# ShuangXieIrene/ssds.pytorch

Hardware: AMD Instinct MI355X
Metric: images/sec (fwd+decode+NMS) SSD-MobileNetV2@512 (higher is better)
Workload: dtype bf16

## Files before the change

### ssds.pytorch_amd/csrc/ssdk_mbk.hip

```cpp
#include "ssdk_common.h"
#include "ssdk_flow_common.h"
#include "ssdk_scan.h"

namespace ssdk {

struct MbkParams {
  const u16* x;
  u16* y;
  const unsigned char* img;
  int N, H, W, Ho, Wo, Cin, Chid, Cout, residual;
  int pairs, halves;
  unsigned items;
  unsigned long long* dbg;
  unsigned wave_mask, pair_mask;
};

template <int KS, int NW, int NCHW, int NFO>
struct MbkGeo {
  static constexpr int NP = (NCHW + 1) / 2;
  static constexpr int PAIR_KB = 2 * KS + NFO;
  static constexpr int MISC_KB = (NCHW * 384 + 1023) / 1024;
  static constexpr int m_be = 0, m_wd = NCHW * 64, m_bd = NCHW * (64 + 288);
  static constexpr int SPB_KB = 2;
  static_assert(NFO * 128 <= SPB_KB * 1024, "projection BN block");
  __host__ __device__ static size_t weights(int halves) { return (size_t)halves * NW * NP * PAIR_KB * 1024; }
  __host__ __device__ static size_t misc_off(int halves) { return weights(halves); }
  __host__ __device__ static size_t spb_off(int halves) { return misc_off(halves) + (size_t)NW * MISC_KB * 1024; }
  __host__ __device__ static size_t bytes(int halves) { return spb_off(halves) + (size_t)halves * SPB_KB * 1024; }
};

template <int S, int NS>
struct MbkItem {
  static constexpr int NXS = NS * S;
  static constexpr int NR = S + 3;
};

template <int S, int NS, int KS, int NW, int NCHW, int NFO>
struct MbkLds {
  using G = MbkGeo<KS, NW, NCHW, NFO>;
  using I = MbkItem<S, NS>;
  static constexpr int FT = 2 * NS * NFO;
  static constexpr int XF = FT % 5 == 0 ? 5 : (FT % 8 == 0 ? 8 : 4);
  static_assert(FT % XF == 0, "exchange rounds");
  static constexpr int xt = 0;
  static constexpr int misc = xt + I::NR * I::NXS * KS * 1024;
  static constexpr int spb = misc + NW * G::MISC_KB * 1024;
  static constexpr int xch = spb + G::SPB_KB * 1024;
  static constexpr int bytes = xch + NW * XF * 1024;
};

__device__ __forceinline__ void mbk_mfma_guard() {
  __builtin_amdgcn_sched_barrier(0);
  asm volatile("s_nop 15\n\ts_nop 3" ::: "memory");
  __builtin_amdgcn_sched_barrier(0);
}
__device__ __forceinline__ void mbk_valu_guard() {
  __builtin_amdgcn_sched_barrier(0);
  asm volatile("s_nop 3" ::: "memory");
  __builtin_amdgcn_sched_barrier(0);
}
__device__ __forceinline__ u32 fl_from_left2(u32 cur, u32 prev) {
  const int old = __builtin_amdgcn_update_dpp(0, (int)prev, 0x121, 0xf, 0xf, true);
  return (u32)__builtin_amdgcn_update_dpp(old, (int)cur, 0x111, 0xf, 0xf, false);
}
__device__ __forceinline__ u32 fl_from_right2(u32 cur, u32 next) {
  const int old = __builtin_amdgcn_update_dpp(0, (int)next, 0x12f, 0xf, 0xf, true);
  return (u32)__builtin_amdgcn_update_dpp(old, (int)cur, 0x101, 0xf, 0xf, false);
}

template <int DT, int S, int NS, int KS, int NW, int NCHW, int NFO, bool DBG = false>
__global__ __launch_bounds__(64 * NW, 2) void mbk_kernel(const MbkParams p) {
  using L = MbkLds<S, NS, KS, NW, NCHW, NFO>;
  using G = MbkGeo<KS, NW, NCHW, NFO>;
  using I = MbkItem<S, NS>;
  constexpr int NR = I::NR, NXS = I::NXS, NE = NR * NXS;
  constexpr int XF = L::XF, FT = L::FT, NP = G::NP, PAIR_KB = G::PAIR_KB;
  constexpr int NO = 2 * NS;
  constexpr bool ODD = (NCHW & 1) != 0;
  constexpr int ROUNDS = FT / XF;
  extern __shared__ __attribute__((aligned(16))) unsigned char smem[];
  const u32 tid = threadIdx.x, lane = tid & 63u;
  const u32 fr = lane & 15u, fg = lane >> 4;
  const int wv = __builtin_amdgcn_readfirstlane((int)(tid >> 6));
  const int Cin = p.Cin, Cout = p.Cout, H = p.H, W = p.W, Ho = p.Ho, Wo = p.Wo;

  const u32 item = blockIdx.x;
  const int half = (int)(item % (u32)p.halves);
  const u32 rem = item / (u32)p.halves;
  const int n = (int)(rem / (u32)p.pairs), rp = (int)(rem % (u32)p.pairs);
  const int oy0 = 2 * rp;
  const int iy0 = S * oy0 - 1;
  const int co_base = half * 16 * NFO;
  const u16* ximg = p.x + (size_t)n * H * W * Cin;
  const bool stamp = p.dbg != nullptr && blockIdx.x == 0 && tid == 0;
  if (stamp) p.dbg[0] = __builtin_readcyclecounter();

  const u32x4* wimg = reinterpret_cast<const u32x4*>(p.img + ((size_t)(half * NW + wv) * NP) * ((size_t)PAIR_KB * 1024)) + lane;
  u32x4 wa[KS], wb[KS];
#pragma unroll
  for (int ks = 0; ks < KS; ++ks) {
    wa[ks] = wimg[(size_t)ks * 64];
    wb[ks] = wimg[(size_t)(KS + ks) * 64];
  }

  for (int e = wv; e < NE; e += NW) {
    const int r = e / NXS, xs = e % NXS;
    int iy = iy0 + r;
    iy = iy < 0 ? 0 : (iy > H - 1 ? H - 1 : iy);
    const int col = S == 1 ? 16 * xs + (int)fr : 2 * (16 * (xs >> 1) + (int)fr) + (xs & 1);
    const u16* src = ximg + ((size_t)iy * W + col) * Cin + fg * 8;
#pragma unroll
    for (int ks = 0; ks < KS; ++ks)
      __builtin_amdgcn_global_load_lds((glb_u8*)(src + ks * 32), (lds_u8*)(smem + L::xt + (e * KS + ks) * 1024), 16, 0, 0);
  }
  {
    const unsigned char* src = p.img + G::misc_off(p.halves) + (size_t)wv * (G::MISC_KB * 1024) + lane * 16;
#pragma unroll
    for (int k = 0; k < G::MISC_KB; ++k)
      __builtin_amdgcn_global_load_lds((glb_u8*)(src + k * 1024), (lds_u8*)(smem + L::misc + (wv * G::MISC_KB + k) * 1024), 16, 0, 0);
  }
  if (wv == 0) {
    const unsigned char* src = p.img + G::spb_off(p.halves) + (size_t)half * (G::SPB_KB * 1024) + lane * 16;
#pragma unroll
    for (int k = 0; k < G::SPB_KB; ++k)
      __builtin_amdgcn_global_load_lds((glb_u8*)(src + k * 1024), (lds_u8*)(smem + L::spb + k * 1024), 16, 0, 0);
  }
  asm volatile("s_waitcnt vmcnt(0)" ::: "memory");
  __syncthreads();
  if (stamp) p.dbg[1] = __builtin_readcyclecounter();

  fl_f2 hi[NR];
#pragma unroll
  for (int r = 0; r < NR; ++r) {
    const float k = ((unsigned)(iy0 + r) < (unsigned)H) ? kFlSixth : 0.f;
    hi[r] = fl_f2{k, k};
  }

  f32x4 yacc[NO][NFO];
#pragma unroll
  for (int o = 0; o < NO; ++o)
#pragma unroll
    for (int f = 0; f < NFO; ++f) yacc[o][f] = f32x4{0.f, 0.f, 0.f, 0.f};

  const unsigned char* xt = smem + L::xt + lane * 16;
  const unsigned char* mc = smem + L::misc + wv * (G::MISC_KB * 1024);

  auto chunk = [&](int c, const u32x4 (&w)[KS], u32 (&dout)[NO][2]) {
    const f32x4 bv = *reinterpret_cast<const f32x4*>(mc + G::m_be + (c * 4 + (int)fg) * 16);
    f32x4 e[NE];
#pragma unroll
    for (int i = 0; i < NE; ++i) e[i] = bv;
#pragma unroll
    for (int ks = 0; ks < KS; ++ks) {
      u32x4 xf[NE];
#pragma unroll
      for (int i = 0; i < NE; ++i) xf[i] = *reinterpret_cast<const u32x4*>(xt + (i * KS + ks) * 1024);
#pragma unroll
      for (int i = 0; i < NE; ++i) e[i] = fl_mfma<DT>(w[ks], xf[i], e[i]);
    }
    uint2 wt[9];
#pragma unroll
    for (int t = 0; t < 9; ++t) wt[t] = *reinterpret_cast<const uint2*>(mc + G::m_wd + ((c * 9 + t) * 4 + (int)fg) * 8);
    const uint2 bdi = *reinterpret_cast<const uint2*>(mc + G::m_bd + (c * 4 + (int)fg) * 8);
    mbk_mfma_guard();
    u32 ew[NR][NXS][2];
#pragma unroll
    for (int r = 0; r < NR; ++r)
#pragma unroll
      for (int xs = 0; xs < NXS; ++xs) {
        ew[r][xs][0] = fl_unit_pack(e[r * NXS + xs][0], e[r * NXS + xs][1], hi[r]);
        ew[r][xs][1] = fl_unit_pack(e[r * NXS + xs][2], e[r * NXS + xs][3], hi[r]);
      }
#pragma unroll
    for (int o = 0; o < 2; ++o)
#pragma unroll
      for (int j = 0; j < NS; ++j) {
        fl_h2 s[2] = {fl_as_h2(bdi.x), fl_as_h2(bdi.y)};
#pragma unroll
        for (int ky = 0; ky < 3; ++ky) {
          const int r = S * o + ky;
          const uint2 w0 = wt[ky * 3], w1 = wt[ky * 3 + 1], w2 = wt[ky * 3 + 2];
#pragma unroll
          for (int wd = 0; wd < 2; ++wd) {
            u32 tl, tc, tr;
            if constexpr (S == 1) {
              tc = ew[r][j][wd];
              tl = j == 0 ? fl_from_left(tc) : fl_from_left2(tc, ew[r][j > 0 ? j - 1 : 0][wd]);
              tr = j == NS - 1 ? fl_from_right(tc) : fl_from_right2(tc, ew[r][j < NS - 1 ? j + 1 : j][wd]);
            } else {
              const u32 odd = ew[r][2 * j + 1][wd];
              tc = ew[r][2 * j][wd];
              tl = j == 0 ? fl_from_left(odd) : fl_from_left2(odd, ew[r][j > 0 ? 2 * j - 1 : 1][wd]);
              tr = odd;
            }
            const u32 ww0 = wd ? w0.y : w0.x, ww1 = wd ? w1.y : w1.x, ww2 = wd ? w2.y : w2.x;
            s[wd] = __builtin_elementwise_fma(fl_as_h2(tl), fl_as_h2(ww0), s[wd]);
            s[wd] = __builtin_elementwise_fma(fl_as_h2(tc), fl_as_h2(ww1), s[wd]);
            if (ky == 2) s[wd] = fl_fma_clamp01(fl_as_h2(tr), fl_as_h2(ww2), s[wd]);
            else s[wd] = __builtin_elementwise_fma(fl_as_h2(tr), fl_as_h2(ww2), s[wd]);
          }
        }
        dout[o * NS + j][0] = fl_as_u32(s[0]);
        dout[o * NS + j][1] = fl_as_u32(s[1]);
      }
  };

  constexpr int FH = NFO / 2;
  for (int t = 0; t < NP; ++t) {
    const u32x4* wp = wimg + (size_t)t * (PAIR_KB * 64);
    const bool last = t == NP - 1;
    const u32x4* wn = wimg + (size_t)(last ? t : t + 1) * (PAIR_KB * 64);
    u32 d0[NO][2], d1[NO][2];
    u32x4 wf0[FH], wf1[NFO - FH];
#pragma unroll
    for (int f = 0; f < FH; ++f) wf0[f] = wp[(size_t)(2 * KS + f) * 64];
    chunk(2 * t, wa, d0);
    __builtin_amdgcn_sched_barrier(0);
    u32x4 na[KS];
#pragma unroll
    for (int ks = 0; ks < KS; ++ks) na[ks] = wn[(size_t)ks * 64];
#pragma unroll
    for (int f = FH; f < NFO; ++f) wf1[f - FH] = wp[(size_t)(2 * KS + f) * 64];
    if (!(ODD && last)) {
      chunk(2 * t + 1, wb, d1);
    } else {
#pragma unroll
      for (int o = 0; o < NO; ++o) d1[o][0] = d1[o][1] = 0u;
    }
    __builtin_amdgcn_sched_barrier(0);
    u32x4 nb[KS];
#pragma unroll
    for (int ks = 0; ks < KS; ++ks) nb[ks] = wn[(size_t)(KS + ks) * 64];
    u32x4 db[NO];
#pragma unroll
    for (int o = 0; o < NO; ++o) db[o] = u32x4{d0[o][0], d0[o][1], d1[o][0], d1[o][1]};
    if constexpr (DBG) {
      if (!((p.pair_mask >> t) & 1u) || !((p.wave_mask >> wv) & 1u)) {
#pragma unroll
        for (int o = 0; o < NO; ++o) db[o] = u32x4{0u, 0u, 0u, 0u};
      }
    }
    mbk_valu_guard();
#pragma unroll
    for (int f = 0; f < NFO; ++f)
#pragma unroll
      for (int o = 0; o < NO; ++o)
        yacc[o][f] = fl_mfma<SSDK_F16>(f < FH ? wf0[f < FH ? f : 0] : wf1[f >= FH ? f - FH : 0], db[o], yacc[o][f]);
    __builtin_amdgcn_sched_barrier(0);
#pragma unroll
    for (int ks = 0; ks < KS; ++ks) {
      wa[ks] = na[ks];
      wb[ks] = nb[ks];
    }
  }
  if (stamp) p.dbg[2] = __builtin_readcyclecounter();

  unsigned char* xb = smem + L::xch;
  const unsigned char* spb = smem + L::spb;
  constexpr int GPW = (XF + NW - 1) / NW;
  uint2 resv[ROUNDS][GPW];
#pragma unroll
  for (int R = 0; R < ROUNDS; ++R)
#pragma unroll
    for (int gg = 0; gg < GPW; ++gg) {
      const int g = wv + gg * NW, q = R * XF + g, oj = q / NFO, f = q % NFO;
      const int oy = oy0 + oj / NS, ox = 16 * (oj % NS) + (int)fr, co = co_base + f * 16 + (int)fg * 4;
      resv[R][gg] = make_uint2(0u, 0u);
      if (S == 1 && p.residual && g < XF && oy < Ho && co < Cout)
        resv[R][gg] = *reinterpret_cast<const uint2*>(ximg + ((size_t)oy * W + ox) * Cin + co);
    }
#pragma unroll
  for (int R = 0; R < ROUNDS; ++R) {
#pragma unroll
    for (int g = 0; g < XF; ++g) {
      const int q = R * XF + g, oj = q / NFO, f = q % NFO;
      *reinterpret_cast<f32x4*>(xb + ((wv * XF + g) * 64 + (int)lane) * 16) = yacc[oj][f];
    }
    __syncthreads();
#pragma unroll
    for (int gg = 0; gg < GPW; ++gg) {
      const int g = wv + gg * NW;
      if (g < XF) {
        const int q = R * XF + g, oj = q / NFO, f = q % NFO;
        f32x4 y = *reinterpret_cast<const f32x4*>(xb + ((0 * XF + g) * 64 + (int)lane) * 16);
#pragma unroll
        for (int w2 = 1; w2 < NW; ++w2) {
          const f32x4 t2 = *reinterpret_cast<const f32x4*>(xb + ((w2 * XF + g) * 64 + (int)lane) * 16);
          y = y + t2;
        }
        const int oy = oy0 + oj / NS, ox = 16 * (oj % NS) + (int)fr;
        const int co = co_base + f * 16 + (int)fg * 4;
        if (oy < Ho && co < Cout) {
          const f32x4 spv = *reinterpret_cast<const f32x4*>(spb + (f * 4 + (int)fg) * 32);
          const f32x4 bpv = *reinterpret_cast<const f32x4*>(spb + (f * 4 + (int)fg) * 32 + 16);
          u32 h01 = fl_pack2<DT>(fmaf(y[0], spv[0], bpv[0]), fmaf(y[1], spv[1], bpv[1]));
          u32 h23 = fl_pack2<DT>(fmaf(y[2], spv[2], bpv[2]), fmaf(y[3], spv[3], bpv[3]));
          if (S == 1 && p.residual) {
            const uint2 xr = resv[R][gg];
            h01 = fl_pack2<DT>(fl_from16<DT>(h01 & 0xffffu) + fl_from16<DT>(xr.x & 0xffffu), fl_from16<DT>(h01 >> 16) + fl_from16<DT>(xr.x >> 16));
            h23 = fl_pack2<DT>(fl_from16<DT>(h23 & 0xffffu) + fl_from16<DT>(xr.y & 0xffffu), fl_from16<DT>(h23 >> 16) + fl_from16<DT>(xr.y >> 16));
          }
          u16* yrow = p.y + (((size_t)n * Ho + oy) * Wo + ox) * Cout;
          *reinterpret_cast<uint2*>(yrow + co) = make_uint2(h01, h23);
        }
      }
    }
    if (R + 1 < ROUNDS) __syncthreads();
  }
  if (stamp) p.dbg[3] = __builtin_readcyclecounter();
}

template <int DT, int S, int NS, int KS, int NW, int NCHW, int NFO, bool DBG = false>
static void mbk_launch(const MbkParams& p, hipStream_t stream) {
  constexpr int lds = MbkLds<S, NS, KS, NW, NCHW, NFO>::bytes;
  static_assert(lds <= 160 * 1024, "LDS");
  (void)hipFuncSetAttribute(reinterpret_cast<const void*>(&mbk_kernel<DT, S, NS, KS, NW, NCHW, NFO, DBG>),
                            hipFuncAttributeMaxDynamicSharedMemorySize, lds);
  hipLaunchKernelGGL((mbk_kernel<DT, S, NS, KS, NW, NCHW, NFO, DBG>), dim3(p.items), dim3(64 * NW), lds, stream, p);
}

constexpr int kMbkNW = 4;
struct MbkInst {
  int s, ns, ks, nchw, nfo;
};
static const MbkInst kMbkInst[] = {{1, 1, 5, 15, 10}, {2, 1, 3, 9, 10}, {1, 2, 2, 6, 4}, {1, 2, 2, 6, 6}, {1, 2, 3, 9, 6},
                                   {2, 2, 1, 3, 4}, {1, 4, 1, 3, 2}};

static int mbk_find(int stride, int Wo, int Cin, int Chid, int Cout, int nw, int* halves) {
  if (nw != kMbkNW || Cin % 32 || Chid % 16 || Cout % 16 || Wo % 16) return -1;
  const int ks = Cin / 32, nch = Chid / 16, nchw = (nch + nw - 1) / nw, ns = Wo / 16;
  for (int i = 0; i < (int)(sizeof(kMbkInst) / sizeof(kMbkInst[0])); ++i) {
    const MbkInst& k = kMbkInst[i];
    if (k.s == stride && k.ns == ns && k.ks == ks && k.nchw == nchw && Cout % (16 * k.nfo) == 0) {
      if (halves) *halves = Cout / (16 * k.nfo);
      return i;
    }
  }
  return -1;
}

static size_t mbk_bytes(int inst, int halves) {
  switch (inst) {
    case 0: return MbkGeo<5, kMbkNW, 15, 10>::bytes(halves);
    case 1: return MbkGeo<3, kMbkNW, 9, 10>::bytes(halves);
    case 2: return MbkGeo<2, kMbkNW, 6, 4>::bytes(halves);
    case 3: return MbkGeo<2, kMbkNW, 6, 6>::bytes(halves);
    case 4: return MbkGeo<3, kMbkNW, 9, 6>::bytes(halves);
    case 5: return MbkGeo<1, kMbkNW, 3, 4>::bytes(halves);
    case 6: return MbkGeo<1, kMbkNW, 3, 2>::bytes(halves);
  }
  return 0;
}

template <int DT>
static void mbk_dispatch(const MbkParams& p, int inst, hipStream_t stream) {
  const bool dbg = p.wave_mask != ~0u || p.pair_mask != ~0u;
  switch (inst) {
    case 0: dbg ? mbk_launch<DT, 1, 1, 5, kMbkNW, 15, 10, true>(p, stream) : mbk_launch<DT, 1, 1, 5, kMbkNW, 15, 10>(p, stream); break;
    case 1: mbk_launch<DT, 2, 1, 3, kMbkNW, 9, 10>(p, stream); break;
    case 2: mbk_launch<DT, 1, 2, 2, kMbkNW, 6, 4>(p, stream); break;
    case 3: mbk_launch<DT, 1, 2, 2, kMbkNW, 6, 6>(p, stream); break;
    case 4: mbk_launch<DT, 1, 2, 3, kMbkNW, 9, 6>(p, stream); break;
    case 5: mbk_launch<DT, 2, 2, 1, kMbkNW, 3, 4>(p, stream); break;
    case 6: mbk_launch<DT, 1, 4, 1, kMbkNW, 3, 2>(p, stream); break;
  }
}

int launch_mbk(const ssdk_mbconv_desc* d, hipStream_t stream) {
  static const int env = getenv("SSDK_MBK") ? atoi(getenv("SSDK_MBK")) : 1;
  const int variant = d->variant;
  if ((!env && variant != 3) || (variant != 0 && variant != 3)) return 1;
  if (d->stem || !d->w_image || d->image_nw < 1 || (d->stride != 1 && d->stride != 2)) return 1;
  const int Ho = (d->H + 2 - 3) / d->stride + 1, Wo = (d->W + 2 - 3) / d->stride + 1;
  if (d->W != Wo * d->stride) return 1;
  int halves = 0;
  const int inst = mbk_find(d->stride, Wo, d->Cin, d->Chid, d->Cout, d->image_nw, &halves);
  if (inst < 0 || (size_t)d->w_image_bytes < mbk_bytes(inst, halves) || ((uintptr_t)d->w_image & 15)) return 1;
  if (env != 1 && variant != 3 && !((env >> (inst + 1)) & 1)) return 1;
  const int pairs = (Ho + 1) / 2;
  const long items = (long)halves * d->N * pairs;
  constexpr int env_min = 256;
  if (items < env_min && variant != 3) return 1;
  MbkParams p;
  p.x = (const u16*)d->x;
  p.y = (u16*)d->y;
  p.img = (const unsigned char*)d->w_image;
  p.N = d->N;
  p.H = d->H;
  p.W = d->W;
  p.Ho = Ho;
  p.Wo = Wo;
  p.Cin = d->Cin;
  p.Chid = d->Chid;
  p.Cout = d->Cout;
  p.residual = d->residual;
  p.pairs = pairs;
  p.halves = halves;
  p.items = (unsigned)items;
  p.dbg = nullptr;
  p.wave_mask = p.pair_mask = ~0u;
  if (const char* m = getenv("SSDK_MBK_MASKS")) {
    unsigned a = ~0u, b = ~0u;
    if (sscanf(m, "%x,%x", &a, &b) == 2) {
      p.wave_mask = a;
      p.pair_mask = b;
    }
  }
  static const int env_dbg = getenv("SSDK_MB_DBG") ? atoi(getenv("SSDK_MB_DBG")) : 0;
  static unsigned long long* dbg_dev = nullptr;
  if (env_dbg) {
    if (!dbg_dev) (void)hipMalloc(&dbg_dev, 8 * sizeof(unsigned long long));
    p.dbg = dbg_dev;
  }
  if (d->dtype == SSDK_BF16) mbk_dispatch<SSDK_BF16>(p, inst, stream);
  else mbk_dispatch<SSDK_F16>(p, inst, stream);
  if (env_dbg) {
    unsigned long long h[4];
    (void)hipStreamSynchronize(stream);
    (void)hipMemcpy(h, dbg_dev, sizeof(h), hipMemcpyDeviceToHost);
    fprintf(stderr, "[mbk dbg] Cin=%d Chid=%d Cout=%d s=%d W=%d items=%ld : setup %llu loop %llu exchange %llu\n", d->Cin, d->Chid,
            d->Cout, d->stride, d->W, items, h[1] - h[0], h[2] - h[1], h[3] - h[2]);
  }
  return 0;
}

}

extern "C" size_t ssdk_mbk_image_bytes(int Cin, int Chid, int Cout, int stride, int Wo, int nw, int* nfo) {
  int halves = 0;
  const int inst = ssdk::mbk_find(stride, Wo, Cin, Chid, Cout, nw, &halves);
  if (inst < 0) return 0;
  if (nfo) *nfo = ssdk::kMbkInst[inst].nfo;
  return ssdk::mbk_bytes(inst, halves);
}
```

Baseline: 65130.

## Make MobileNet block kernel persistent with double-buffered input tile prefetch

```diff
diff --git a/ssds.pytorch_amd/csrc/ssdk_mbk.hip b/ssds.pytorch_amd/csrc/ssdk_mbk.hip
--- a/ssds.pytorch_amd/csrc/ssdk_mbk.hip
+++ b/ssds.pytorch_amd/csrc/ssdk_mbk.hip
@@ -11,6 +11,7 @@
   int N, H, W, Ho, Wo, Cin, Chid, Cout, residual;
   int pairs, halves;
   unsigned items;
+  unsigned grid;
   unsigned long long* dbg;
   unsigned wave_mask, pair_mask;
 };
@@ -39,15 +40,57 @@
 struct MbkLds {
   using G = MbkGeo<KS, NW, NCHW, NFO>;
   using I = MbkItem<S, NS>;
+  static constexpr int kHalfCu = 80 * 1024;
   static constexpr int FT = 2 * NS * NFO;
-  static constexpr int XF = FT % 5 == 0 ? 5 : (FT % 8 == 0 ? 8 : 4);
+  static constexpr int XF1 = FT % 5 == 0 ? 5 : (FT % 8 == 0 ? 8 : 4);
+  static constexpr int xt_bytes = I::NR * I::NXS * KS * 1024;
+  static constexpr int fixed = (NW * G::MISC_KB + G::SPB_KB) * 1024;
+  static constexpr bool two_xf1 = 2 * xt_bytes + fixed + NW * XF1 * 1024 <= kHalfCu;
+  static constexpr bool two_xf4 = FT % 4 == 0 && 2 * xt_bytes + fixed + NW * 4 * 1024 <= kHalfCu;
+  static constexpr int NXB = (two_xf1 || two_xf4) ? 2 : 1;
+  static constexpr int XF = two_xf1 ? XF1 : (two_xf4 ? 4 : XF1);
   static_assert(FT % XF == 0, "exchange rounds");
   static constexpr int xt = 0;
-  static constexpr int misc = xt + I::NR * I::NXS * KS * 1024;
+  static constexpr int misc = xt + NXB * xt_bytes;
   static constexpr int spb = misc + NW * G::MISC_KB * 1024;
   static constexpr int xch = spb + G::SPB_KB * 1024;
   static constexpr int bytes = xch + NW * XF * 1024;
+  static_assert(bytes <= kHalfCu, "two workgroups per CU");
+  static_assert(NXB == 2 || FT / XF >= 2, "one tile: the refill runs under the exchange rounds behind the first");
 };
+
+struct MbkWalk {
+  u32 unit, half, halves, units, step;
+  bool single;
+  __host__ __device__ MbkWalk(u32 items, u32 halves_, u32 grid, u32 wg)
+      : halves(halves_), units(items / halves_), step(grid), single(grid >= items) {
+    unit = single ? wg / halves : wg;
+    half = single ? wg % halves : 0u;
+  }
+  __host__ __device__ bool valid() const { return unit < units; }
+  __host__ __device__ bool peek(u32& nu, u32& nh) const {
+    nu = unit;
+    nh = half + 1u;
+    if (nh == halves) {
+      nh = 0u;
+      nu = unit + step;
+    }
+    return !single && nu < units;
+  }
+};
+
+__device__ __forceinline__ u32 mbk_here(u32 v) {
+  asm volatile("" : "+v"(v));
+  return v;
+}
+
+__device__ __forceinline__ void mbk_glds16(const void* gsrc, u32 lds_dst) {
+  u32 keep;
+  asm volatile("s_mov_b32 %0, m0\n\ts_mov_b32 m0, %2\n\ts_nop 0\n\tglobal_load_lds_dwordx4 %1, off\n\ts_mov_b32 m0, %0"
+               : "=&s"(keep)
+               : "v"(gsrc), "s"(__builtin_amdgcn_readfirstlane((int)lds_dst))
+               : "memory");
+}
 
 __device__ __forceinline__ void mbk_mfma_guard() {
   __builtin_amdgcn_sched_barrier(0);
@@ -74,249 +117,289 @@
   using G = MbkGeo<KS, NW, NCHW, NFO>;
   using I = MbkItem<S, NS>;
   constexpr int NR = I::NR, NXS = I::NXS, NE = NR * NXS;
-  constexpr int XF = L::XF, FT = L::FT, NP = G::NP, PAIR_KB = G::PAIR_KB;
+  constexpr int XF = L::XF, FT = L::FT, NP = G::NP, PAIR_KB = G::PAIR_KB, NXB = L::NXB;
   constexpr int NO = 2 * NS;
   constexpr bool ODD = (NCHW & 1) != 0;
   constexpr int ROUNDS = FT / XF;
   extern __shared__ __attribute__((aligned(16))) unsigned char smem[];
   const u32 tid = threadIdx.x, lane = tid & 63u;
-  const u32 fr = lane & 15u, fg = lane >> 4;
+  const u32 fg = lane >> 4;
   const int wv = __builtin_amdgcn_readfirstlane((int)(tid >> 6));
   const int Cin = p.Cin, Cout = p.Cout, H = p.H, W = p.W, Ho = p.Ho, Wo = p.Wo;
-
-  const u32 item = blockIdx.x;
-  const int half = (int)(item % (u32)p.halves);
-  const u32 rem = item / (u32)p.halves;
-  const int n = (int)(rem / (u32)p.pairs), rp = (int)(rem % (u32)p.pairs);
-  const int oy0 = 2 * rp;
-  const int iy0 = S * oy0 - 1;
-  const int co_base = half * 16 * NFO;
-  const u16* ximg = p.x + (size_t)n * H * W * Cin;
-  const bool stamp = p.dbg != nullptr && blockIdx.x == 0 && tid == 0;
-  if (stamp) p.dbg[0] = __builtin_readcyclecounter();
-
-  const u32x4* wimg = reinterpret_cast<const u32x4*>(p.img + ((size_t)(half * NW + wv) * NP) * ((size_t)PAIR_KB * 1024)) + lane;
+  const u32 lds0 = (u32)(uintptr_t)(lds_u8*)smem;
+
+  MbkWalk wk(p.items, (u32)p.halves, p.grid, blockIdx.x);
+  if (!wk.valid()) return;
+  const bool stamp0 = p.dbg != nullptr && blockIdx.x == 0 && tid == 0;
+  if (stamp0) p.dbg[0] = __builtin_readcyclecounter();
+
+  auto wimg_of = [&](u32 h) {
+    return reinterpret_cast<const u32x4*>(p.img + ((size_t)((int)h * NW + wv) * NP) * ((size_t)PAIR_KB * 1024)) + lane;
+  };
+  auto tile_dma = [&](u32 u, int buf) {
+    const int un = (int)(u / (u32)p.pairs), urp = (int)(u % (u32)p.pairs);
+    const int uiy0 = S * 2 * urp - 1;
+    const u16* uimg = p.x + (size_t)un * H * W * Cin;
+    const u32 dfr = mbk_here(lane) & 15u, dfg = mbk_here(lane) >> 4;
+    for (int e = wv; e < NE; e += NW) {
+      const int r = e / NXS, xs = e % NXS;
+      int iy = uiy0 + r;
+      iy = iy < 0 ? 0 : (iy > H - 1 ? H - 1 : iy);
+      const int col = S == 1 ? 16 * xs + (int)dfr : 2 * (16 * (xs >> 1) + (int)dfr) + (xs & 1);
+      const u16* src = uimg + ((size_t)iy * W + col) * Cin + dfg * 8;
+#pragma unroll
+      for (int ks = 0; ks < KS; ++ks) mbk_glds16(src + ks * 32, lds0 + (u32)(L::xt + buf * L::xt_bytes + (e * KS + ks) * 1024));
+    }
+  };
+  auto spb_dma = [&](u32 h) {
+    if (wv == 0) {
+      const unsigned char* src = p.img + G::spb_off(p.halves) + (size_t)h * (G::SPB_KB * 1024) + lane * 16;
+#pragma unroll
+      for (int k = 0; k < G::SPB_KB; ++k) mbk_glds16(src + k * 1024, lds0 + (u32)(L::spb + k * 1024));
+    }
+  };
+
+  const u32x4* wimg = wimg_of(wk.half);
   u32x4 wa[KS], wb[KS];
 #pragma unroll
   for (int ks = 0; ks < KS; ++ks) {
     wa[ks] = wimg[(size_t)ks * 64];
     wb[ks] = wimg[(size_t)(KS + ks) * 64];
   }
-
-  for (int e = wv; e < NE; e += NW) {
-    const int r = e / NXS, xs = e % NXS;
-    int iy = iy0 + r;
-    iy = iy < 0 ? 0 : (iy > H - 1 ? H - 1 : iy);
-    const int col = S == 1 ? 16 * xs + (int)fr : 2 * (16 * (xs >> 1) + (int)fr) + (xs & 1);
-    const u16* src = ximg + ((size_t)iy * W + col) * Cin + fg * 8;
-#pragma unroll
-    for (int ks = 0; ks < KS; ++ks)
-      __builtin_amdgcn_global_load_lds((glb_u8*)(src + ks * 32), (lds_u8*)(smem + L::xt + (e * KS + ks) * 1024), 16, 0, 0);
-  }
+  tile_dma(wk.unit, 0);
   {
     const unsigned char* src = p.img + G::misc_off(p.halves) + (size_t)wv * (G::MISC_KB * 1024) + lane * 16;
 #pragma unroll
-    for (int k = 0; k < G::MISC_KB; ++k)
-      __builtin_amdgcn_global_load_lds((glb_u8*)(src + k * 1024), (lds_u8*)(smem + L::misc + (wv * G::MISC_KB + k) * 1024), 16, 0, 0);
-  }
-  if (wv == 0) {
-    const unsigned char* src = p.img + G::spb_off(p.halves) + (size_t)half * (G::SPB_KB * 1024) + lane * 16;
-#pragma unroll
-    for (int k = 0; k < G::SPB_KB; ++k)
-      __builtin_amdgcn_global_load_lds((glb_u8*)(src + k * 1024), (lds_u8*)(smem + L::spb + k * 1024), 16, 0, 0);
-  }
+    for (int k = 0; k < G::MISC_KB; ++k) mbk_glds16(src + k * 1024, lds0 + (u32)(L::misc + (wv * G::MISC_KB + k) * 1024));
+  }
+  spb_dma(wk.half);
   asm volatile("s_waitcnt vmcnt(0)" ::: "memory");
   __syncthreads();
-  if (stamp) p.dbg[1] = __builtin_readcyclecounter();
-
-  fl_f2 hi[NR];
-#pragma unroll
-  for (int r = 0; r < NR; ++r) {
-    const float k = ((unsigned)(iy0 + r) < (unsigned)H) ? kFlSixth : 0.f;
-    hi[r] = fl_f2{k, k};
-  }
-
-  f32x4 yacc[NO][NFO];
-#pragma unroll
-  for (int o = 0; o < NO; ++o)
-#pragma unroll
-    for (int f = 0; f < NFO; ++f) yacc[o][f] = f32x4{0.f, 0.f, 0.f, 0.f};
-
-  const unsigned char* xt = smem + L::xt + lane * 16;
+
   const unsigned char* mc = smem + L::misc + wv * (G::MISC_KB * 1024);
-
-  auto chunk = [&](int c, const u32x4 (&w)[KS], u32 (&dout)[NO][2]) {
-    const f32x4 bv = *reinterpret_cast<const f32x4*>(mc + G::m_be + (c * 4 + (int)fg) * 16);
-    f32x4 e[NE];
-#pragma unroll
-    for (int i = 0; i < NE; ++i) e[i] = bv;
-#pragma unroll
-    for (int ks = 0; ks < KS; ++ks) {
-      u32x4 xf[NE];
-#pragma unroll
-      for (int i = 0; i < NE; ++i) xf[i] = *reinterpret_cast<const u32x4*>(xt + (i * KS + ks) * 1024);
-#pragma unroll
-      for (int i = 0; i < NE; ++i) e[i] = fl_mfma<DT>(w[ks], xf[i], e[i]);
-    }
-    uint2 wt[9];
-#pragma unroll
-    for (int t = 0; t < 9; ++t) wt[t] = *reinterpret_cast<const uint2*>(mc + G::m_wd + ((c * 9 + t) * 4 + (int)fg) * 8);
-    const uint2 bdi = *reinterpret_cast<const uint2*>(mc + G::m_bd + (c * 4 + (int)fg) * 8);
-    mbk_mfma_guard();
-    u32 ew[NR][NXS][2];
-#pragma unroll
-    for (int r = 0; r < NR; ++r)
-#pragma unroll
-      for (int xs = 0; xs < NXS; ++xs) {
-        ew[r][xs][0] = fl_unit_pack(e[r * NXS + xs][0], e[r * NXS + xs][1], hi[r]);
-        ew[r][xs][1] = fl_unit_pack(e[r * NXS + xs][2], e[r * NXS + xs][3], hi[r]);
-      }
-#pragma unroll
-    for (int o = 0; o < 2; ++o)
-#pragma unroll
-      for (int j = 0; j < NS; ++j) {
-        fl_h2 s[2] = {fl_as_h2(bdi.x), fl_as_h2(bdi.y)};
-#pragma unroll
-        for (int ky = 0; ky < 3; ++ky) {
-          const int r = S * o + ky;
-          const uint2 w0 = wt[ky * 3], w1 = wt[ky * 3 + 1], w2 = wt[ky * 3 + 2];
-#pragma unroll
-          for (int wd = 0; wd < 2; ++wd) {
-            u32 tl, tc, tr;
-            if constexpr (S == 1) {
-              tc = ew[r][j][wd];
-              tl = j == 0 ? fl_from_left(tc) : fl_from_left2(tc, ew[r][j > 0 ? j - 1 : 0][wd]);
-              tr = j == NS - 1 ? fl_from_right(tc) : fl_from_right2(tc, ew[r][j < NS - 1 ? j + 1 : j][wd]);
-            } else {
-              const u32 odd = ew[r][2 * j + 1][wd];
-              tc = ew[r][2 * j][wd];
-              tl = j == 0 ? fl_from_left(odd) : fl_from_left2(odd, ew[r][j > 0 ? 2 * j - 1 : 1][wd]);
-              tr = odd;
+  const unsigned char* spb = smem + L::spb;
+  unsigned char* xb = smem + L::xch;
+  int cur = 0;
+
+  for (u32 it = 0;; ++it) {
+    const bool stamp = stamp0 && it < 2u;
+    unsigned long long* dbg = p.dbg + 4 * it;
+    if (stamp && it) dbg[0] = __builtin_readcyclecounter();
+    u32 nunit, nhalf;
+    const bool more = wk.peek(nunit, nhalf);
+    const bool refill = more && nunit != wk.unit;
+    const int half = (int)wk.half;
+    const int n = (int)(wk.unit / (u32)p.pairs), rp = (int)(wk.unit % (u32)p.pairs);
+    const int oy0 = 2 * rp;
+    const int iy0 = S * oy0 - 1;
+    const int co_base = half * 16 * NFO;
+    const u16* ximg = p.x + (size_t)n * H * W * Cin;
+    const u32x4* wnext = more ? wimg_of(nhalf) : wimg;
+    if (NXB == 2 && refill) tile_dma(nunit, cur ^ 1);
+    if (stamp) dbg[1] = __builtin_readcyclecounter();
+
+    fl_f2 hi[NR];
+#pragma unroll
+    for (int r = 0; r < NR; ++r) {
+      const float k = ((unsigned)(iy0 + r) < (unsigned)H) ? kFlSixth : 0.f;
+      hi[r] = fl_f2{k, k};
+    }
+
+    f32x4 yacc[NO][NFO];
+#pragma unroll
+    for (int o = 0; o < NO; ++o)
+#pragma unroll
+      for (int f = 0; f < NFO; ++f) yacc[o][f] = f32x4{0.f, 0.f, 0.f, 0.f};
+
+    const unsigned char* xt = smem + L::xt + cur * L::xt_bytes + lane * 16;
+
+    auto chunk = [&](int c, const u32x4 (&w)[KS], u32 (&dout)[NO][2]) {
+      const f32x4 bv = *reinterpret_cast<const f32x4*>(mc + G::m_be + (c * 4 + (int)fg) * 16);
+      f32x4 e[NE];
+#pragma unroll
+      for (int i = 0; i < NE; ++i) e[i] = bv;
+#pragma unroll
+      for (int ks = 0; ks < KS; ++ks) {
+        u32x4 xf[NE];
+#pragma unroll
+        for (int i = 0; i < NE; ++i) xf[i] = *reinterpret_cast<const u32x4*>(xt + (i * KS + ks) * 1024);
+#pragma unroll
+        for (int i = 0; i < NE; ++i) e[i] = fl_mfma<DT>(w[ks], xf[i], e[i]);
+      }
+      uint2 wt[9];
+#pragma unroll
+      for (int t = 0; t < 9; ++t) wt[t] = *reinterpret_cast<const uint2*>(mc + G::m_wd + ((c * 9 + t) * 4 + (int)fg) * 8);
+      const uint2 bdi = *reinterpret_cast<const uint2*>(mc + G::m_bd + (c * 4 + (int)fg) * 8);
+      mbk_mfma_guard();
+      u32 ew[NR][NXS][2];
+#pragma unroll
+      for (int r = 0; r < NR; ++r)
+#pragma unroll
+        for (int xs = 0; xs < NXS; ++xs) {
+          ew[r][xs][0] = fl_unit_pack(e[r * NXS + xs][0], e[r * NXS + xs][1], hi[r]);
+          ew[r][xs][1] = fl_unit_pack(e[r * NXS + xs][2], e[r * NXS + xs][3], hi[r]);
+        }
+#pragma unroll
+      for (int o = 0; o < 2; ++o)
+#pragma unroll
+        for (int j = 0; j < NS; ++j) {
+          fl_h2 s[2] = {fl_as_h2(bdi.x), fl_as_h2(bdi.y)};
+#pragma unroll
+          for (int ky = 0; ky < 3; ++ky) {
+            const int r = S * o + ky;
+            const uint2 w0 = wt[ky * 3], w1 = wt[ky * 3 + 1], w2 = wt[ky * 3 + 2];
+#pragma unroll
+            for (int wd = 0; wd < 2; ++wd) {
+              u32 tl, tc, tr;
+              if constexpr (S == 1) {
+                tc = ew[r][j][wd];
+                tl = j == 0 ? fl_from_left(tc) : fl_from_left2(tc, ew[r][j > 0 ? j - 1 : 0][wd]);
+                tr = j == NS - 1 ? fl_from_right(tc) : fl_from_right2(tc, ew[r][j < NS - 1 ? j + 1 : j][wd]);
+              } else {
+                const u32 odd = ew[r][2 * j + 1][wd];
+                tc = ew[r][2 * j][wd];
+                tl = j == 0 ? fl_from_left(odd) : fl_from_left2(odd, ew[r][j > 0 ? 2 * j - 1 : 1][wd]);
+                tr = odd;
+              }
+              const u32 ww0 = wd ? w0.y : w0.x, ww1 = wd ? w1.y : w1.x, ww2 = wd ? w2.y : w2.x;
+              s[wd] = __builtin_elementwise_fma(fl_as_h2(tl), fl_as_h2(ww0), s[wd]);
+              s[wd] = __builtin_elementwise_fma(fl_as_h2(tc), fl_as_h2(ww1), s[wd]);
+              if (ky == 2) s[wd] = fl_fma_clamp01(fl_as_h2(tr), fl_as_h2(ww2), s[wd]);
+              else s[wd] = __builtin_elementwise_fma(fl_as_h2(tr), fl_as_h2(ww2), s[wd]);
             }
-            const u32 ww0 = wd ? w0.y : w0.x, ww1 = wd ? w1.y : w1.x, ww2 = wd ? w2.y : w2.x;
-            s[wd] = __builtin_elementwise_fma(fl_as_h2(tl), fl_as_h2(ww0), s[wd]);
-            s[wd] = __builtin_elementwise_fma(fl_as_h2(tc), fl_as_h2(ww1), s[wd]);
-            if (ky == 2) s[wd] = fl_fma_clamp01(fl_as_h2(tr), fl_as_h2(ww2), s[wd]);
-            else s[wd] = __builtin_elementwise_fma(fl_as_h2(tr), fl_as_h2(ww2), s[wd]);
+          }
+          dout[o * NS + j][0] = fl_as_u32(s[0]);
+          dout[o * NS + j][1] = fl_as_u32(s[1]);
+        }
+    };
+
+    constexpr int FH = NFO / 2;
+    for (int t = 0; t < NP; ++t) {
+      const u32x4* wp = wimg + (size_t)t * (PAIR_KB * 64);
+      const bool last = t == NP - 1;
+      const u32x4* wn = last ? wnext : wimg + (size_t)(t + 1) * (PAIR_KB * 64);
+      u32 d0[NO][2], d1[NO][2];
+      u32x4 wf0[FH], wf1[NFO - FH];
+#pragma unroll
+      for (int f = 0; f < FH; ++f) wf0[f] = wp[(size_t)(2 * KS + f) * 64];
+      chunk(2 * t, wa, d0);
+      __builtin_amdgcn_sched_barrier(0);
+      u32x4 na[KS];
+#pragma unroll
+      for (int ks = 0; ks < KS; ++ks) na[ks] = wn[(size_t)ks * 64];
+#pragma unroll
+      for (int f = FH; f < NFO; ++f) wf1[f - FH] = wp[(size_t)(2 * KS + f) * 64];
+      if (!(ODD && last)) {
+        chunk(2 * t + 1, wb, d1);
+      } else {
+#pragma unroll
+        for (int o = 0; o < NO; ++o) d1[o][0] = d1[o][1] = 0u;
+      }
+      __builtin_amdgcn_sched_barrier(0);
+      u32x4 nb[KS];
+#pragma unroll
+      for (int ks = 0; ks < KS; ++ks) nb[ks] = wn[(size_t)(KS + ks) * 64];
+      u32x4 db[NO];
+#pragma unroll
+      for (int o = 0; o < NO; ++o) db[o] = u32x4{d0[o][0], d0[o][1], d1[o][0], d1[o][1]};
+      if constexpr (DBG) {
+        if (!((p.pair_mask >> t) & 1u) || !((p.wave_mask >> wv) & 1u)) {
+#pragma unroll
+          for (int o = 0; o < NO; ++o) db[o] = u32x4{0u, 0u, 0u, 0u};
+        }
+      }
+      mbk_valu_guard();
+#pragma unroll
+      for (int f = 0; f < NFO; ++f)
+#pragma unroll
+        for (int o = 0; o < NO; ++o)
+          yacc[o][f] = fl_mfma<SSDK_F16>(f < FH ? wf0[f < FH ? f : 0] : wf1[f >= FH ? f - FH : 0], db[o], yacc[o][f]);
+      __builtin_amdgcn_sched_barrier(0);
+#pragma unroll
+      for (int ks = 0; ks < KS; ++ks) {
+        wa[ks] = na[ks];
+        wb[ks] = nb[ks];
+      }
+    }
+    asm volatile("s_waitcnt vmcnt(%0)" ::"n"(KS) : "memory");
+    if (stamp) dbg[2] = __builtin_readcyclecounter();
+
+    constexpr int GPW = (XF + NW - 1) / NW;
+    const u32 xlane = mbk_here(lane), xfr = xlane & 15u, xfg = xlane >> 4;
+    uint2 resv[ROUNDS][GPW];
+#pragma unroll
+    for (int R = 0; R < ROUNDS; ++R)
+#pragma unroll
+      for (int gg = 0; gg < GPW; ++gg) {
+        const int g = wv + gg * NW, q = R * XF + g, oj = q / NFO, f = q % NFO;
+        const int oy = oy0 + oj / NS, ox = 16 * (oj % NS) + (int)xfr, co = co_base + f * 16 + (int)xfg * 4;
+        resv[R][gg] = make_uint2(0u, 0u);
+        if (S == 1 && p.residual && g < XF && oy < Ho && co < Cout)
+          resv[R][gg] = *reinterpret_cast<const uint2*>(ximg + ((size_t)oy * W + ox) * Cin + co);
+      }
+#pragma unroll
+    for (int R = 0; R < ROUNDS; ++R) {
+#pragma unroll
+      for (int g = 0; g < XF; ++g) {
+        const int q = R * XF + g, oj = q / NFO, f = q % NFO;
+        *reinterpret_cast<f32x4*>(xb + ((wv * XF + g) * 64 + (int)xlane) * 16) = yacc[oj][f];
+      }
+      if (NXB == 1 && R == ROUNDS - 1 && refill) asm volatile("s_waitcnt vmcnt(0)" ::: "memory");
+      __syncthreads();
+      if (S == 1 && R == 0) {
+#pragma unroll
+        for (int r2 = 0; r2 < ROUNDS; ++r2)
+#pragma unroll
+          for (int gg = 0; gg < GPW; ++gg) asm volatile("" ::"v"(resv[r2][gg].x), "v"(resv[r2][gg].y));
+      }
+      if (NXB == 1 && R == 0 && refill) tile_dma(nunit, 0);
+#pragma unroll
+      for (int gg = 0; gg < GPW; ++gg) {
+        const int g = wv + gg * NW;
+        if (g < XF) {
+          const int q = R * XF + g, oj = q / NFO, f = q % NFO;
+          f32x4 y = *reinterpret_cast<const f32x4*>(xb + ((0 * XF + g) * 64 + (int)xlane) * 16);
+#pragma unroll
+          for (int w2 = 1; w2 < NW; ++w2) {
+            const f32x4 t2 = *reinterpret_cast<const f32x4*>(xb + ((w2 * XF + g) * 64 + (int)xlane) * 16);
+            y = y + t2;
+          }
+          const int oy = oy0 + oj / NS, ox = 16 * (oj % NS) + (int)xfr;
+          const int co = co_base + f * 16 + (int)xfg * 4;
+          if (oy < Ho && co < Cout) {
+            const f32x4 spv = *reinterpret_cast<const f32x4*>(spb + (f * 4 + (int)xfg) * 32);
+            const f32x4 bpv = *reinterpret_cast<const f32x4*>(spb + (f * 4 + (int)xfg) * 32 + 16);
+            u32 h01 = fl_pack2<DT>(fmaf(y[0], spv[0], bpv[0]), fmaf(y[1], spv[1], bpv[1]));
+            u32 h23 = fl_pack2<DT>(fmaf(y[2], spv[2], bpv[2]), fmaf(y[3], spv[3], bpv[3]));
+            if (S == 1 && p.residual) {
+              const uint2 xr = resv[R][gg];
+              h01 = fl_pack2<DT>(fl_from16<DT>(h01 & 0xffffu) + fl_from16<DT>(xr.x & 0xffffu), fl_from16<DT>(h01 >> 16) + fl_from16<DT>(xr.x >> 16));
+              h23 = fl_pack2<DT>(fl_from16<DT>(h23 & 0xffffu) + fl_from16<DT>(xr.y & 0xffffu), fl_from16<DT>(h23 >> 16) + fl_from16<DT>(xr.y >> 16));
+            }
+            u16* yrow = p.y + (((size_t)n * Ho + oy) * Wo + ox) * Cout;
+            *reinterpret_cast<uint2*>(yrow + co) = make_uint2(h01, h23);
           }
         }
-        dout[o * NS + j][0] = fl_as_u32(s[0]);
-        dout[o * NS + j][1] = fl_as_u32(s[1]);
-      }
-  };
-
-  constexpr int FH = NFO / 2;
-  for (int t = 0; t < NP; ++t) {
-    const u32x4* wp = wimg + (size_t)t * (PAIR_KB * 64);
-    const bool last = t == NP - 1;
-    const u32x4* wn = wimg + (size_t)(last ? t : t + 1) * (PAIR_KB * 64);
-    u32 d0[NO][2], d1[NO][2];
-    u32x4 wf0[FH], wf1[NFO - FH];
-#pragma unroll
-    for (int f = 0; f < FH; ++f) wf0[f] = wp[(size_t)(2 * KS + f) * 64];
-    chunk(2 * t, wa, d0);
-    __builtin_amdgcn_sched_barrier(0);
-    u32x4 na[KS];
-#pragma unroll
-    for (int ks = 0; ks < KS; ++ks) na[ks] = wn[(size_t)ks * 64];
-#pragma unroll
-    for (int f = FH; f < NFO; ++f) wf1[f - FH] = wp[(size_t)(2 * KS + f) * 64];
-    if (!(ODD && last)) {
-      chunk(2 * t + 1, wb, d1);
-    } else {
-#pragma unroll
-      for (int o = 0; o < NO; ++o) d1[o][0] = d1[o][1] = 0u;
-    }
-    __builtin_amdgcn_sched_barrier(0);
-    u32x4 nb[KS];
-#pragma unroll
-    for (int ks = 0; ks < KS; ++ks) nb[ks] = wn[(size_t)(KS + ks) * 64];
-    u32x4 db[NO];
-#pragma unroll
-    for (int o = 0; o < NO; ++o) db[o] = u32x4{d0[o][0], d0[o][1], d1[o][0], d1[o][1]};
-    if constexpr (DBG) {
-      if (!((p.pair_mask >> t) & 1u) || !((p.wave_mask >> wv) & 1u)) {
-#pragma unroll
-        for (int o = 0; o < NO; ++o) db[o] = u32x4{0u, 0u, 0u, 0u};
-      }
-    }
-    mbk_valu_guard();
-#pragma unroll
-    for (int f = 0; f < NFO; ++f)
-#pragma unroll
-      for (int o = 0; o < NO; ++o)
-        yacc[o][f] = fl_mfma<SSDK_F16>(f < FH ? wf0[f < FH ? f : 0] : wf1[f >= FH ? f - FH : 0], db[o], yacc[o][f]);
-    __builtin_amdgcn_sched_barrier(0);
-#pragma unroll
-    for (int ks = 0; ks < KS; ++ks) {
-      wa[ks] = na[ks];
-      wb[ks] = nb[ks];
-    }
-  }
-  if (stamp) p.dbg[2] = __builtin_readcyclecounter();
-
-  unsigned char* xb = smem + L::xch;
-  const unsigned char* spb = smem + L::spb;
-  constexpr int GPW = (XF + NW - 1) / NW;
-  uint2 resv[ROUNDS][GPW];
-#pragma unroll
-  for (int R = 0; R < ROUNDS; ++R)
-#pragma unroll
-    for (int gg = 0; gg < GPW; ++gg) {
-      const int g = wv + gg * NW, q = R * XF + g, oj = q / NFO, f = q % NFO;
-      const int oy = oy0 + oj / NS, ox = 16 * (oj % NS) + (int)fr, co = co_base + f * 16 + (int)fg * 4;
-      resv[R][gg] = make_uint2(0u, 0u);
-      if (S == 1 && p.residual && g < XF && oy < Ho && co < Cout)
-        resv[R][gg] = *reinterpret_cast<const uint2*>(ximg + ((size_t)oy * W + ox) * Cin + co);
-    }
-#pragma unroll
-  for (int R = 0; R < ROUNDS; ++R) {
-#pragma unroll
-    for (int g = 0; g < XF; ++g) {
-      const int q = R * XF + g, oj = q / NFO, f = q % NFO;
-      *reinterpret_cast<f32x4*>(xb + ((wv * XF + g) * 64 + (int)lane) * 16) = yacc[oj][f];
-    }
+      }
+      if (R + 1 < ROUNDS) __syncthreads();
+    }
+    if (stamp) dbg[3] = __builtin_readcyclecounter();
+    if (!more) break;
     __syncthreads();
-#pragma unroll
-    for (int gg = 0; gg < GPW; ++gg) {
-      const int g = wv + gg * NW;
-      if (g < XF) {
-        const int q = R * XF + g, oj = q / NFO, f = q % NFO;
-        f32x4 y = *reinterpret_cast<const f32x4*>(xb + ((0 * XF + g) * 64 + (int)lane) * 16);
-#pragma unroll
-        for (int w2 = 1; w2 < NW; ++w2) {
-          const f32x4 t2 = *reinterpret_cast<const f32x4*>(xb + ((w2 * XF + g) * 64 + (int)lane) * 16);
-          y = y + t2;
-        }
-        const int oy = oy0 + oj / NS, ox = 16 * (oj % NS) + (int)fr;
-        const int co = co_base + f * 16 + (int)fg * 4;
-        if (oy < Ho && co < Cout) {
-          const f32x4 spv = *reinterpret_cast<const f32x4*>(spb + (f * 4 + (int)fg) * 32);
-          const f32x4 bpv = *reinterpret_cast<const f32x4*>(spb + (f * 4 + (int)fg) * 32 + 16);
-          u32 h01 = fl_pack2<DT>(fmaf(y[0], spv[0], bpv[0]), fmaf(y[1], spv[1], bpv[1]));
-          u32 h23 = fl_pack2<DT>(fmaf(y[2], spv[2], bpv[2]), fmaf(y[3], spv[3], bpv[3]));
-          if (S == 1 && p.residual) {
-            const uint2 xr = resv[R][gg];
-            h01 = fl_pack2<DT>(fl_from16<DT>(h01 & 0xffffu) + fl_from16<DT>(xr.x & 0xffffu), fl_from16<DT>(h01 >> 16) + fl_from16<DT>(xr.x >> 16));
-            h23 = fl_pack2<DT>(fl_from16<DT>(h23 & 0xffffu) + fl_from16<DT>(xr.y & 0xffffu), fl_from16<DT>(h23 >> 16) + fl_from16<DT>(xr.y >> 16));
-          }
-          u16* yrow = p.y + (((size_t)n * Ho + oy) * Wo + ox) * Cout;
-          *reinterpret_cast<uint2*>(yrow + co) = make_uint2(h01, h23);
-        }
-      }
-    }
-    if (R + 1 < ROUNDS) __syncthreads();
-  }
-  if (stamp) p.dbg[3] = __builtin_readcyclecounter();
+    if (nhalf != wk.half) spb_dma(nhalf);
+    if (nunit != wk.unit) cur ^= NXB - 1;
+    wk.unit = nunit;
+    wk.half = nhalf;
+    wimg = wnext;
+  }
 }
 
 template <int DT, int S, int NS, int KS, int NW, int NCHW, int NFO, bool DBG = false>
 static void mbk_launch(const MbkParams& p, hipStream_t stream) {
   constexpr int lds = MbkLds<S, NS, KS, NW, NCHW, NFO>::bytes;
-  static_assert(lds <= 160 * 1024, "LDS");
   (void)hipFuncSetAttribute(reinterpret_cast<const void*>(&mbk_kernel<DT, S, NS, KS, NW, NCHW, NFO, DBG>),
                             hipFuncAttributeMaxDynamicSharedMemorySize, lds);
-  hipLaunchKernelGGL((mbk_kernel<DT, S, NS, KS, NW, NCHW, NFO, DBG>), dim3(p.items), dim3(64 * NW), lds, stream, p);
+  hipLaunchKernelGGL((mbk_kernel<DT, S, NS, KS, NW, NCHW, NFO, DBG>), dim3(p.grid), dim3(64 * NW), lds, stream, p);
 }
 
 constexpr int kMbkNW = 4;
@@ -397,6 +480,21 @@
   p.pairs = pairs;
   p.halves = halves;
   p.items = (unsigned)items;
+  static const int persist = getenv("SSDK_MBK_PERSIST") ? atoi(getenv("SSDK_MBK_PERSIST")) : 1;
+  p.grid = p.items;
+  if (persist) {
+    static int cus = 0;
+    if (!cus) {
+      int dev = 0;
+      (void)hipGetDevice(&dev);
+      if (hipDeviceGetAttribute(&cus, hipDeviceAttributeMultiprocessorCount, dev) != hipSuccess || cus <= 0) cus = 256;
+    }
+    if (p.grid > 2u * (unsigned)cus) p.grid = 2u * (unsigned)cus;
+  }
+  if (const char* g = getenv("SSDK_MBK_GRID")) {
+    const int v = atoi(g);
+    if (v > 0) p.grid = (unsigned)v < p.items ? (unsigned)v : p.items;
+  }
   p.dbg = nullptr;
   p.wave_mask = p.pair_mask = ~0u;
   if (const char* m = getenv("SSDK_MBK_MASKS")) {
@@ -410,20 +508,40 @@
   static unsigned long long* dbg_dev = nullptr;
   if (env_dbg) {
     if (!dbg_dev) (void)hipMalloc(&dbg_dev, 8 * sizeof(unsigned long long));
+    (void)hipMemsetAsync(dbg_dev, 0, 8 * sizeof(unsigned long long), stream);
     p.dbg = dbg_dev;
   }
   if (d->dtype == SSDK_BF16) mbk_dispatch<SSDK_BF16>(p, inst, stream);
   else mbk_dispatch<SSDK_F16>(p, inst, stream);
   if (env_dbg) {
-    unsigned long long h[4];
+    unsigned long long h[8];
     (void)hipStreamSynchronize(stream);
     (void)hipMemcpy(h, dbg_dev, sizeof(h), hipMemcpyDeviceToHost);
     fprintf(stderr, "[mbk dbg] Cin=%d Chid=%d Cout=%d s=%d W=%d items=%ld : setup %llu loop %llu exchange %llu\n", d->Cin, d->Chid,
             d->Cout, d->stride, d->W, items, h[1] - h[0], h[2] - h[1], h[3] - h[2]);
+    if (h[7])
+      fprintf(stderr, "[mbk dbg]   grid=%u, second item: wait %llu setup %llu loop %llu exchange %llu\n", p.grid, h[4] - h[3], h[5] - h[4],
+              h[6] - h[5], h[7] - h[6]);
   }
   return 0;
 }
 
+}
+
+extern "C" int ssdk_mbk_item_walk(unsigned items, unsigned halves, unsigned grid, unsigned wg, unsigned* out, int cap) {
+  if (!halves || !grid || items % halves) return -1;
+  ssdk::MbkWalk wk(items, halves, grid, wg);
+  int n = 0;
+  if (!wk.valid()) return 0;
+  for (;;) {
+    if (out && n < cap) out[n] = wk.unit * halves + wk.half;
+    ++n;
+    unsigned nu, nh;
+    if (!wk.peek(nu, nh)) break;
+    wk.unit = nu;
+    wk.half = nh;
+  }
+  return n;
 }
 
 extern "C" size_t ssdk_mbk_image_bytes(int Cin, int Chid, int Cout, int stride, int Wo, int nw, int* nfo) {
```

After: 64510. No clear change (-0.9%).
